# google-research/rigl

Hardware: AMD Instinct MI355X
Metric: images/sec/node, ResNet-50 80% ERK RigL step (higher is better)
Workload: dtype bf16

## Files before the change

rigl_amd/csrc/bn.hip:

```cpp
#include "common.hpp"

namespace rigl {
namespace kbn {

constexpr int THREADS = 256;
constexpr int MAX_PARTS = 512;

__device__ __forceinline__ float bf_lo(uint32_t w) { return __uint_as_float(w << 16); }
__device__ __forceinline__ float bf_hi(uint32_t w) { return __uint_as_float(w & 0xFFFF0000u); }
__device__ __forceinline__ uint32_t f2bf(float f) {
  uint32_t u = __float_as_uint(f);
  if ((u & 0x7FFFFFFFu) > 0x7F800000u) return (u >> 16) | 0x40u;
  u += 0x7FFFu + ((u >> 16) & 1u);
  return u >> 16;
}
typedef __attribute__((ext_vector_type(2))) __bf16 bf16x2_t;
typedef __attribute__((ext_vector_type(2))) float f32x2_t;
__device__ __forceinline__ uint32_t pack2(float a, float b) {
  const f32x2_t v = {a, b};
  return __builtin_bit_cast(uint32_t, __builtin_convertvector(v, bf16x2_t));
}
__device__ __forceinline__ void unpack8(const uint4& v, float f[8]) {
  f[0] = bf_lo(v.x); f[1] = bf_hi(v.x); f[2] = bf_lo(v.y); f[3] = bf_hi(v.y);
  f[4] = bf_lo(v.z); f[5] = bf_hi(v.z); f[6] = bf_lo(v.w); f[7] = bf_hi(v.w);
}

typedef unsigned int u32x4_t __attribute__((ext_vector_type(4)));
__device__ __forceinline__ void st16(uint16_t* p, const uint4& v, int nt) {
  if (nt) { const u32x4_t t = {v.x, v.y, v.z, v.w}; __builtin_nontemporal_store(t, reinterpret_cast<u32x4_t*>(p)); }
  else *reinterpret_cast<uint4*>(p) = v;
}
__device__ __forceinline__ uint4 ld16(const uint16_t* p, int nt) {
  if (nt > 1) { const u32x4_t t = __builtin_nontemporal_load(reinterpret_cast<const u32x4_t*>(p)); return make_uint4(t.x, t.y, t.z, t.w); }
  return *reinterpret_cast<const uint4*>(p);
}

struct Geom {
  int nt;
  int il;
  int64_t M;
  int C, cg;
  int tpr, rpb;
  int parts;
  int64_t rows_per_part;
  int fixed;
};

__device__ __forceinline__ void ld8f(const float* __restrict__ p, float (&o)[8]) {
  const float4 a = *reinterpret_cast<const float4*>(p), b = *reinterpret_cast<const float4*>(p + 4);
  o[0] = a.x; o[1] = a.y; o[2] = a.z; o[3] = a.w; o[4] = b.x; o[5] = b.y; o[6] = b.z; o[7] = b.w;
}

__device__ __forceinline__ float pivot3(float a, float b, float c) { return fmaxf(fminf(a, b), fminf(fmaxf(a, b), c)); }

template <int MODE, bool RELU, int MSK>
__global__ __launch_bounds__(THREADS) void k_reduce(Geom G, const uint16_t* __restrict__ x, const uint16_t* __restrict__ y,
                                                    const uint8_t* __restrict__ mbits,
                                                    const uint16_t* __restrict__ dy, const float* __restrict__ mean,
                                                    const float* __restrict__ invstd, const float* __restrict__ scale,
                                                    const float* __restrict__ shift, float* __restrict__ partial) {
  __shared__ float red[THREADS][17];
  const int tx = threadIdx.x % G.tpr, ty = threadIdx.x / G.tpr;
  const int cgi = blockIdx.y * G.tpr + tx;
  const bool c_ok = cgi < G.cg;
  const int64_t r0 = (int64_t)blockIdx.x * G.rows_per_part;
  int64_t r1 = r0 + G.rows_per_part;
  if (r1 > G.M) r1 = G.M;
  float q0[8], q1[8], mu[8], is[8], sc[8], sh[8];
#pragma unroll
  for (int j = 0; j < 8; ++j) { q0[j] = q1[j] = 0.f; mu[j] = is[j] = sc[j] = sh[j] = 0.f; }
  if (MODE == 1 && c_ok) {
#pragma unroll
    for (int j = 0; j < 8; ++j) {
      mu[j] = mean[cgi * 8 + j]; is[j] = invstd[cgi * 8 + j];
      if (RELU && MSK == 0) { sc[j] = scale[cgi * 8 + j]; sh[j] = shift[cgi * 8 + j]; }
    }
  }
  if (MODE == 0 && c_ok) {
    float pa[8], pb[8], pc[8];
    unpack8(*reinterpret_cast<const uint4*>(x + (int64_t)cgi * 8), pa);
    unpack8(*reinterpret_cast<const uint4*>(x + (G.M / 2) * G.C + (int64_t)cgi * 8), pb);
    unpack8(*reinterpret_cast<const uint4*>(x + (G.M - 1) * G.C + (int64_t)cgi * 8), pc);
#pragma unroll
    for (int j = 0; j < 8; ++j) mu[j] = pivot3(pa[j], pb[j], pc[j]);
  }
  if (c_ok) {
    const int64_t rb = G.il ? (int64_t)blockIdx.x * G.rpb + ty : r0 + ty, re = G.il ? G.M : r1;
    const int64_t rstep = G.il ? (int64_t)G.parts * G.rpb : (int64_t)G.rpb;
#pragma unroll 2
    for (int64_t r = rb; r < re; r += rstep) {
      const int64_t off = r * G.C + (int64_t)cgi * 8;
      float xv[8];
      unpack8(*reinterpret_cast<const uint4*>(x + off), xv);
      if (MODE == 0) {
#pragma unroll
        for (int j = 0; j < 8; ++j) { const float d = xv[j] - mu[j]; q0[j] += d; q1[j] = fmaf(d, d, q1[j]); }
      } else {
        float dv[8], yv[8];
        unpack8(*reinterpret_cast<const uint4*>(dy + off), dv);
        uint32_t mb = 0u;
        if (RELU && MSK == 1) unpack8(*reinterpret_cast<const uint4*>(y + off), yv);
        if (RELU && MSK == 2) mb = mbits[r * G.cg + cgi];
#pragma unroll
        for (int j = 0; j < 8; ++j) {
          bool on = true;
          if (RELU) on = MSK == 1 ? (yv[j] > 0.f) : (MSK == 2 ? ((mb >> j) & 1u) != 0u : (fmaf(xv[j], sc[j], sh[j]) > 0.f));
          const float dz = on ? dv[j] : 0.f;
          q0[j] += dz;
          q1[j] = fmaf(dz, (xv[j] - mu[j]) * is[j], q1[j]);
        }
      }
    }
  }
  float own[16];
#pragma unroll
  for (int j = 0; j < 8; ++j) { own[j] = q0[j]; own[8 + j] = q1[j]; red[threadIdx.x][j] = q0[j]; red[threadIdx.x][8 + j] = q1[j]; }
  __syncthreads();
  for (int s = G.rpb >> 1; s > 0; s >>= 1) {
    if (ty < s) {
      float oth[16];
#pragma unroll
      for (int j = 0; j < 16; ++j) oth[j] = red[threadIdx.x + s * G.tpr][j];
#pragma unroll
      for (int j = 0; j < 16; ++j) own[j] += oth[j];
      if (s > 1) {
#pragma unroll
        for (int j = 0; j < 16; ++j) red[threadIdx.x][j] = own[j];
      }
    }
    if (s > 1) __syncthreads();
  }
  if (ty == 0 && c_ok) {
    float* p = partial + ((int64_t)blockIdx.x * 2) * G.C + cgi * 8;
#pragma unroll
    for (int j = 0; j < 8; ++j) { p[j] = own[j]; p[G.C + j] = own[8 + j]; }
  }
}

template <int CL>
__device__ __forceinline__ void sum_partials(const Geom& G, const float* __restrict__ partial, double& s0, double& s1,
                                             int& c, bool& leader) {
  constexpr int PL = THREADS / CL;
  __shared__ double acc[2][PL][CL + 1];
  const int cl = threadIdx.x % CL, pl = threadIdx.x / CL;
  c = blockIdx.x * CL + cl;
  double a0 = 0.0, a1 = 0.0;
  if (c < G.C) {
#ifndef RIGL_BN_FIN_FLIGHT
#define RIGL_BN_FIN_FLIGHT 16
#endif
    constexpr int FLIGHT = RIGL_BN_FIN_FLIGHT;
    for (int p0 = pl; p0 < G.parts; p0 += PL * FLIGHT) {
      float v0[FLIGHT], v1[FLIGHT];
#pragma unroll
      for (int j = 0; j < FLIGHT; ++j) {
        const int p = p0 + j * PL;
        const int pc = p < G.parts ? p : G.parts - 1;
        const float l0 = partial[((int64_t)pc * 2) * G.C + c], l1 = partial[((int64_t)pc * 2 + 1) * G.C + c];
        v0[j] = p < G.parts ? l0 : 0.f;
        v1[j] = p < G.parts ? l1 : 0.f;
      }
#pragma unroll
      for (int j = 0; j < FLIGHT; ++j) { a0 += (double)v0[j]; a1 += (double)v1[j]; }
    }
  }
  acc[0][pl][cl] = a0; acc[1][pl][cl] = a1;
  __syncthreads();
  leader = pl == 0 && c < G.C;
  s0 = s1 = 0.0;
  if constexpr (CL == 1) {
    __shared__ double acc2[2][16];
    if (threadIdx.x < 16) {
      double t0 = 0.0, t1 = 0.0;
#pragma unroll
      for (int k = 0; k < 16; ++k) { t0 += acc[0][threadIdx.x * 16 + k][0]; t1 += acc[1][threadIdx.x * 16 + k][0]; }
      acc2[0][threadIdx.x] = t0; acc2[1][threadIdx.x] = t1;
    }
    __syncthreads();
    if (leader) {
#pragma unroll
      for (int k = 0; k < 16; ++k) { s0 += acc2[0][k]; s1 += acc2[1][k]; }
    }
  } else if (leader) {
#pragma unroll 8
    for (int k = 0; k < PL; ++k) { s0 += acc[0][k][cl]; s1 += acc[1][k][cl]; }
  }
}

template <int CL>
__global__ __launch_bounds__(THREADS) void k_fwd_finalize(Geom G, const float* __restrict__ partial,
                                                           const uint16_t* __restrict__ x ,
                                                           const float* __restrict__ gamma, const float* __restrict__ beta,
                                                           float* __restrict__ running_mean, float* __restrict__ running_var,
                                                           float momentum, float eps, float* __restrict__ save_mean,
                                                           float* __restrict__ save_invstd, float* __restrict__ scale,
                                                           float* __restrict__ shift) {
  double s0, s1; int c; bool leader;
  sum_partials<CL>(G, partial, s0, s1, c, leader);
  if (!leader) return;
  const double m = (double)G.M;
  double k = 0.0;
  if (x) {
    const float a = __uint_as_float((uint32_t)x[c] << 16), b = __uint_as_float((uint32_t)x[(G.M / 2) * G.C + c] << 16),
                e = __uint_as_float((uint32_t)x[(G.M - 1) * G.C + c] << 16);
    k = (double)pivot3(a, b, e);
  }
  const double dm = s0 / m;
  const double mean = k + dm;
  double var = s1 / m - dm * dm;
  if (var < 0.0) var = 0.0;
  const float invstd = (float)(1.0 / sqrt(var + (double)eps));
  save_mean[c] = (float)mean;
  save_invstd[c] = invstd;
  const float sc = gamma[c] * invstd;
  scale[c] = sc;
  shift[c] = beta[c] - (float)mean * sc;
  if (running_mean) {
    const double unbiased = G.M > 1 ? var * m / (m - 1.0) : var;
    running_mean[c] = (1.f - momentum) * running_mean[c] + momentum * (float)mean;
    running_var[c] = (1.f - momentum) * running_var[c] + momentum * (float)unbiased;
  }
}

template <bool RELU, bool HAS_RES>
__global__ __launch_bounds__(THREADS) void k_fwd_apply(Geom G, const uint16_t* __restrict__ x, const uint16_t* __restrict__ res,
                                                        const float* __restrict__ scale, const float* __restrict__ shift,
                                                        uint16_t* __restrict__ y, uint8_t* __restrict__ mbits) {
  extern __shared__ __attribute__((aligned(16))) float prm[];
  const bool fixed = G.fixed != 0;
  float psc[8], psh[8];
  if (fixed) {
    const int c0 = (int)(((int64_t)blockIdx.x * THREADS + threadIdx.x) % G.cg) * 8;
    ld8f(scale + c0, psc); ld8f(shift + c0, psh);
  } else {
    for (int i = threadIdx.x; i < G.C; i += THREADS) { prm[i] = scale[i]; prm[G.C + i] = shift[i]; }
    __syncthreads();
  }
  const int64_t total = G.M * G.cg;
  const int64_t stride = (int64_t)gridDim.x * THREADS;
  for (int64_t i = (int64_t)blockIdx.x * THREADS + threadIdx.x; i < total; i += stride) {
    if (!fixed) {
      const int cgi = (int)(i % G.cg);
#pragma unroll
      for (int j = 0; j < 8; ++j) { psc[j] = prm[cgi * 8 + j]; psh[j] = prm[G.C + cgi * 8 + j]; }
    }
    float xv[8], rv[8];
    unpack8(ld16(x + i * 8, G.nt), xv);
    if (HAS_RES) unpack8(ld16(res + i * 8, G.nt), rv);
    float o[8];
#pragma unroll
    for (int j = 0; j < 8; ++j) {
      float v = fmaf(xv[j], psc[j], psh[j]);
      if (HAS_RES) v += rv[j];
      o[j] = RELU ? fmaxf(v, 0.f) : v;
    }
    uint4 out;
    out.x = pack2(o[0], o[1]); out.y = pack2(o[2], o[3]); out.z = pack2(o[4], o[5]); out.w = pack2(o[6], o[7]);
    st16(y + i * 8, out, G.nt);
    if (RELU && mbits) {
      uint32_t mb = 0u;
#pragma unroll
      for (int j = 0; j < 8; ++j) mb |= (o[j] > 0.f ? 1u : 0u) << j;
      mbits[i] = (uint8_t)mb;
    }
  }
}

template <int CL>
__global__ __launch_bounds__(THREADS) void k_bwd_finalize(Geom G, const float* __restrict__ partial,
                                                           const float* __restrict__ gamma, const float* __restrict__ invstd,
                                                           float* __restrict__ dgamma, float* __restrict__ dbeta,
                                                           float* __restrict__ coef ) {
  double s0, s1; int c; bool leader;
  sum_partials<CL>(G, partial, s0, s1, c, leader);
  if (!leader) return;
  dbeta[c] = (float)s0;
  dgamma[c] = (float)s1;
  coef[c] = gamma[c] * invstd[c];
  coef[G.C + c] = (float)(s0 / (double)G.M);
  coef[2 * G.C + c] = (float)(s1 / (double)G.M);
}

template <bool RELU, int MSK, bool HAS_DRES>
__global__ __launch_bounds__(THREADS) void k_bwd_apply(Geom G, const uint16_t* __restrict__ x, const uint16_t* __restrict__ y,
                                                        const uint8_t* __restrict__ mbits,
                                                        const uint16_t* __restrict__ dy, const float* __restrict__ mean,
                                                        const float* __restrict__ invstd, const float* __restrict__ scale,
                                                        const float* __restrict__ shift, const float* __restrict__ coef,
                                                        uint16_t* __restrict__ dx, uint16_t* __restrict__ dres) {
  extern __shared__ __attribute__((aligned(16))) float prm[];
  const bool fixed = G.fixed != 0;
  float pm[8], pis[8], pa[8], pb[8], pc[8], psc[8], psh[8];
  if (fixed) {
    const int c0 = (int)(((int64_t)blockIdx.x * THREADS + threadIdx.x) % G.cg) * 8;
    ld8f(mean + c0, pm); ld8f(invstd + c0, pis);
    ld8f(coef + c0, pa); ld8f(coef + G.C + c0, pb); ld8f(coef + 2 * G.C + c0, pc);
    if (RELU && MSK == 0) { ld8f(scale + c0, psc); ld8f(shift + c0, psh); }
  } else {
    for (int i = threadIdx.x; i < G.C; i += THREADS) {
      prm[i] = mean[i]; prm[G.C + i] = invstd[i];
      prm[2 * G.C + i] = coef[i]; prm[3 * G.C + i] = coef[G.C + i]; prm[4 * G.C + i] = coef[2 * G.C + i];
      if (RELU && MSK == 0) { prm[5 * G.C + i] = scale[i]; prm[6 * G.C + i] = shift[i]; }
    }
    __syncthreads();
  }
  const int64_t total = G.M * G.cg;
  const int64_t stride = (int64_t)gridDim.x * THREADS;
  for (int64_t i = (int64_t)blockIdx.x * THREADS + threadIdx.x; i < total; i += stride) {
    if (!fixed) {
      const int c0 = (int)(i % G.cg) * 8;
#pragma unroll
      for (int j = 0; j < 8; ++j) {
        pm[j] = prm[c0 + j]; pis[j] = prm[G.C + c0 + j]; pa[j] = prm[2 * G.C + c0 + j]; pb[j] = prm[3 * G.C + c0 + j];
        pc[j] = prm[4 * G.C + c0 + j];
        if (RELU && MSK == 0) { psc[j] = prm[5 * G.C + c0 + j]; psh[j] = prm[6 * G.C + c0 + j]; }
      }
    }
    float xv[8], dv[8], yv[8];
    unpack8(ld16(x + i * 8, G.nt), xv);
    unpack8(ld16(dy + i * 8, G.nt), dv);
    uint32_t mb = 0u;
    if (RELU && MSK == 1) unpack8(*reinterpret_cast<const uint4*>(y + i * 8), yv);
    if (RELU && MSK == 2) mb = mbits[i];
    float o[8], z[8];
#pragma unroll
    for (int j = 0; j < 8; ++j) {
      bool on = true;
      if (RELU) on = MSK == 1 ? (yv[j] > 0.f) : (MSK == 2 ? ((mb >> j) & 1u) != 0u : (fmaf(xv[j], psc[j], psh[j]) > 0.f));
      const float dz = on ? dv[j] : 0.f;
      o[j] = bn_bwd_dx(dz, xv[j], pm[j], pis[j], pa[j], pb[j], pc[j]);
      z[j] = dz;
    }
    uint4 out;
    out.x = pack2(o[0], o[1]); out.y = pack2(o[2], o[3]); out.z = pack2(o[4], o[5]); out.w = pack2(o[6], o[7]);
    st16(dx + i * 8, out, G.nt);
    if (HAS_DRES) {
      out.x = pack2(z[0], z[1]); out.y = pack2(z[2], z[3]); out.z = pack2(z[4], z[5]); out.w = pack2(z[6], z[7]);
      st16(dres + i * 8, out, G.nt);
    }
  }
}

template <bool RELU>
__global__ __launch_bounds__(THREADS) void k_fwd_apply_pair(Geom G, const uint16_t* __restrict__ x, const uint16_t* __restrict__ x2,
                                                             const float* __restrict__ scale, const float* __restrict__ shift,
                                                             const float* __restrict__ scale2, const float* __restrict__ shift2,
                                                             uint16_t* __restrict__ y, uint8_t* __restrict__ mbits) {
  extern __shared__ __attribute__((aligned(16))) float prm[];
  const bool fixed = G.fixed != 0;
  float p0[8], p1[8], p2[8], p3[8];
  if (fixed) {
    const int c0 = (int)(((int64_t)blockIdx.x * THREADS + threadIdx.x) % G.cg) * 8;
    ld8f(scale + c0, p0); ld8f(shift + c0, p1); ld8f(scale2 + c0, p2); ld8f(shift2 + c0, p3);
  } else {
    for (int i = threadIdx.x; i < G.C; i += THREADS) {
      prm[i] = scale[i]; prm[G.C + i] = shift[i]; prm[2 * G.C + i] = scale2[i]; prm[3 * G.C + i] = shift2[i];
    }
    __syncthreads();
  }
  const int64_t total = G.M * G.cg;
  const int64_t stride = (int64_t)gridDim.x * THREADS;
  for (int64_t i = (int64_t)blockIdx.x * THREADS + threadIdx.x; i < total; i += stride) {
    if (!fixed) {
      const int c0 = (int)(i % G.cg) * 8;
#pragma unroll
      for (int j = 0; j < 8; ++j) { p0[j] = prm[c0 + j]; p1[j] = prm[G.C + c0 + j]; p2[j] = prm[2 * G.C + c0 + j]; p3[j] = prm[3 * G.C + c0 + j]; }
    }
    float xv[8], rv[8];
    unpack8(ld16(x + i * 8, G.nt), xv);
    unpack8(ld16(x2 + i * 8, G.nt), rv);
    float o[8];
#pragma unroll
    for (int j = 0; j < 8; j += 2) {
      const uint32_t pk = pack2(fmaf(rv[j], p2[j], p3[j]), fmaf(rv[j + 1], p2[j + 1], p3[j + 1]));
      float v0 = fmaf(xv[j], p0[j], p1[j]);
      float v1 = fmaf(xv[j + 1], p0[j + 1], p1[j + 1]);
      v0 += bf_lo(pk); v1 += bf_hi(pk);
      o[j] = RELU ? fmaxf(v0, 0.f) : v0;
      o[j + 1] = RELU ? fmaxf(v1, 0.f) : v1;
    }
    uint4 out;
    out.x = pack2(o[0], o[1]); out.y = pack2(o[2], o[3]); out.z = pack2(o[4], o[5]); out.w = pack2(o[6], o[7]);
    st16(y + i * 8, out, G.nt);
    if (RELU && mbits) {
      uint32_t mb = 0u;
#pragma unroll
      for (int j = 0; j < 8; ++j) mb |= (o[j] > 0.f ? 1u : 0u) << j;
      mbits[i] = (uint8_t)mb;
    }
  }
}

__global__ __launch_bounds__(THREADS) void k_reduce_pair(Geom G, const uint16_t* __restrict__ x, const uint16_t* __restrict__ x2,
                                                          const uint8_t* __restrict__ mbits, const uint16_t* __restrict__ dy,
                                                          const float* __restrict__ mean, const float* __restrict__ invstd,
                                                          const float* __restrict__ mean2, const float* __restrict__ invstd2,
                                                          float* __restrict__ partial, float* __restrict__ partial2) {
  __shared__ float red[THREADS][25];
  const int tx = threadIdx.x % G.tpr, ty = threadIdx.x / G.tpr;
  const int cgi = blockIdx.y * G.tpr + tx;
  const bool c_ok = cgi < G.cg;
  const int64_t r0 = (int64_t)blockIdx.x * G.rows_per_part;
  int64_t r1 = r0 + G.rows_per_part;
  if (r1 > G.M) r1 = G.M;
  float q0[8], q1[8], q2[8], mu[8], is[8], mu2[8], is2[8];
#pragma unroll
  for (int j = 0; j < 8; ++j) { q0[j] = q1[j] = q2[j] = 0.f; mu[j] = is[j] = mu2[j] = is2[j] = 0.f; }
  if (c_ok) {
#pragma unroll
    for (int j = 0; j < 8; ++j) {
      mu[j] = mean[cgi * 8 + j]; is[j] = invstd[cgi * 8 + j]; mu2[j] = mean2[cgi * 8 + j]; is2[j] = invstd2[cgi * 8 + j];
    }
    const int64_t rb = G.il ? (int64_t)blockIdx.x * G.rpb + ty : r0 + ty, re = G.il ? G.M : r1;
    const int64_t rstep = G.il ? (int64_t)G.parts * G.rpb : (int64_t)G.rpb;
#pragma unroll 2
    for (int64_t r = rb; r < re; r += rstep) {
      const int64_t off = r * G.C + (int64_t)cgi * 8;
      float xv[8], x2v[8], dv[8];
      unpack8(*reinterpret_cast<const uint4*>(x + off), xv);
      unpack8(*reinterpret_cast<const uint4*>(x2 + off), x2v);
      unpack8(*reinterpret_cast<const uint4*>(dy + off), dv);
      const uint32_t mb = mbits[r * G.cg + cgi];
#pragma unroll
      for (int j = 0; j < 8; ++j) {
        const float dz = ((mb >> j) & 1u) != 0u ? dv[j] : 0.f;
        q0[j] += dz;
        q1[j] = fmaf(dz, (xv[j] - mu[j]) * is[j], q1[j]);
        q2[j] = fmaf(dz, (x2v[j] - mu2[j]) * is2[j], q2[j]);
      }
    }
  }
  float own[24];
#pragma unroll
  for (int j = 0; j < 8; ++j) {
    own[j] = q0[j]; own[8 + j] = q1[j]; own[16 + j] = q2[j];
    red[threadIdx.x][j] = q0[j]; red[threadIdx.x][8 + j] = q1[j]; red[threadIdx.x][16 + j] = q2[j];
  }
  __syncthreads();
  for (int s = G.rpb >> 1; s > 0; s >>= 1) {
    if (ty < s) {
      float oth[24];
#pragma unroll
      for (int j = 0; j < 24; ++j) oth[j] = red[threadIdx.x + s * G.tpr][j];
#pragma unroll
      for (int j = 0; j < 24; ++j) own[j] += oth[j];
      if (s > 1) {
#pragma unroll
        for (int j = 0; j < 24; ++j) red[threadIdx.x][j] = own[j];
      }
    }
    if (s > 1) __syncthreads();
  }
  if (ty == 0 && c_ok) {
    float* p = partial + ((int64_t)blockIdx.x * 2) * G.C + cgi * 8;
    float* p2 = partial2 + ((int64_t)blockIdx.x * 2) * G.C + cgi * 8;
#pragma unroll
    for (int j = 0; j < 8; ++j) {
      p[j] = own[j]; p[G.C + j] = own[8 + j];
      p2[j] = own[j]; p2[G.C + j] = own[16 + j];
    }
  }
}

struct FinSet { const float* partial; const float* gamma; const float* invstd; float* dgamma; float* dbeta; float* coef; };

template <int CL>
__global__ __launch_bounds__(THREADS) void k_bwd_finalize_pair(Geom G, FinSet s0, FinSet s1) {
  const FinSet& f = blockIdx.y == 0 ? s0 : s1;
  double a0, a1; int c; bool leader;
  sum_partials<CL>(G, f.partial, a0, a1, c, leader);
  if (!leader) return;
  f.dbeta[c] = (float)a0;
  f.dgamma[c] = (float)a1;
  f.coef[c] = f.gamma[c] * f.invstd[c];
  f.coef[G.C + c] = (float)(a0 / (double)G.M);
  f.coef[2 * G.C + c] = (float)(a1 / (double)G.M);
}

__global__ __launch_bounds__(THREADS) void k_bwd_apply_pair(Geom G, const uint16_t* __restrict__ x, const uint16_t* __restrict__ x2,
                                                             const uint8_t* __restrict__ mbits, const uint16_t* __restrict__ dy,
                                                             const float* __restrict__ mean, const float* __restrict__ invstd,
                                                             const float* __restrict__ mean2, const float* __restrict__ invstd2,
                                                             const float* __restrict__ coef, const float* __restrict__ coef2,
                                                             uint16_t* __restrict__ dx, uint16_t* __restrict__ dx2) {
  extern __shared__ __attribute__((aligned(16))) float prm[];
  const bool fixed = G.fixed != 0;
  float q[10][8];
  if (fixed) {
    const int c0 = (int)(((int64_t)blockIdx.x * THREADS + threadIdx.x) % G.cg) * 8;
    ld8f(mean + c0, q[0]); ld8f(invstd + c0, q[1]); ld8f(coef + c0, q[2]); ld8f(coef + G.C + c0, q[3]); ld8f(coef + 2 * G.C + c0, q[4]);
    ld8f(mean2 + c0, q[5]); ld8f(invstd2 + c0, q[6]); ld8f(coef2 + c0, q[7]); ld8f(coef2 + G.C + c0, q[8]); ld8f(coef2 + 2 * G.C + c0, q[9]);
  } else {
    for (int i = threadIdx.x; i < G.C; i += THREADS) {
      prm[i] = mean[i]; prm[G.C + i] = invstd[i];
      prm[2 * G.C + i] = coef[i]; prm[3 * G.C + i] = coef[G.C + i]; prm[4 * G.C + i] = coef[2 * G.C + i];
      prm[5 * G.C + i] = mean2[i]; prm[6 * G.C + i] = invstd2[i];
      prm[7 * G.C + i] = coef2[i]; prm[8 * G.C + i] = coef2[G.C + i]; prm[9 * G.C + i] = coef2[2 * G.C + i];
    }
    __syncthreads();
  }
  const int64_t total = G.M * G.cg;
  const int64_t stride = (int64_t)gridDim.x * THREADS;
  for (int64_t i = (int64_t)blockIdx.x * THREADS + threadIdx.x; i < total; i += stride) {
    if (!fixed) {
      const int c0 = (int)(i % G.cg) * 8;
#pragma unroll
      for (int k = 0; k < 10; ++k)
#pragma unroll
        for (int j = 0; j < 8; ++j) q[k][j] = prm[k * G.C + c0 + j];
    }
    float xv[8], x2v[8], dv[8];
    unpack8(ld16(x + i * 8, G.nt), xv);
    unpack8(ld16(x2 + i * 8, G.nt), x2v);
    unpack8(ld16(dy + i * 8, G.nt), dv);
    const uint32_t mb = mbits[i];
    float o[8], o2[8];
#pragma unroll
    for (int j = 0; j < 8; ++j) {
      const float dz = ((mb >> j) & 1u) != 0u ? dv[j] : 0.f;
      const float xh = (xv[j] - q[0][j]) * q[1][j];
      o[j] = q[2][j] * (dz - q[3][j] - xh * q[4][j]);
      const float xh2 = (x2v[j] - q[5][j]) * q[6][j];
      o2[j] = q[7][j] * (dz - q[8][j] - xh2 * q[9][j]);
    }
    uint4 out;
    out.x = pack2(o[0], o[1]); out.y = pack2(o[2], o[3]); out.z = pack2(o[4], o[5]); out.w = pack2(o[6], o[7]);
    st16(dx + i * 8, out, G.nt);
    out.x = pack2(o2[0], o2[1]); out.y = pack2(o2[2], o2[3]); out.z = pack2(o2[4], o2[5]); out.w = pack2(o2[6], o2[7]);
    st16(dx2 + i * 8, out, G.nt);
  }
}

constexpr int INFER_BATCH = 64;
struct InferBatch {
  RiglBnInferItem it[INFER_BATCH];
  int32_t blk_begin[INFER_BATCH + 1];
  int32_t count;
};
__global__ __launch_bounds__(THREADS) void k_infer_params(InferBatch B) {
  int i = 0;
  while (i + 1 < B.count && (int)blockIdx.x >= B.blk_begin[i + 1]) ++i;
  const RiglBnInferItem& t = B.it[i];
  const int c = ((int)blockIdx.x - B.blk_begin[i]) * THREADS + (int)threadIdx.x;
  if (c >= t.c) return;
  const float invstd = (float)(1.0 / sqrt((double)t.moving_variance[c] + (double)t.eps));
  const float sc = t.gamma[c] * invstd;
  t.scale_shift[c] = sc;
  t.scale_shift[t.c + c] = t.beta[c] - t.moving_mean[c] * sc;
}

static Geom make_geom(int64_t m, int c) {
  Geom g;
  g.nt = (int64_t)m * c * 2 >= (int64_t)RIGL_TUNE("bn_nt_mb", 0) * (1 << 20) ? RIGL_TUNE("bn_nt", 2) : 0;
  g.il = RIGL_TUNE("bn_il", 1);
  g.fixed = 0;
  g.M = m; g.C = c; g.cg = c / 8;
  int tpr = 1;
  while (tpr < g.cg && tpr < THREADS) tpr <<= 1;
  g.tpr = tpr; g.rpb = THREADS / tpr;
#ifndef RIGL_BN_ROWS_PER_LANE
#define RIGL_BN_ROWS_PER_LANE 8
#endif
  int64_t parts = (m + (int64_t)g.rpb * RIGL_BN_ROWS_PER_LANE - 1) / ((int64_t)g.rpb * RIGL_BN_ROWS_PER_LANE);
  const int64_t cap = RIGL_TUNE("bn_max_parts", MAX_PARTS);
  if (parts > cap) parts = cap;
  if (parts < 1) parts = 1;
  int64_t rpp = (m + parts - 1) / parts;
  rpp = (rpp + g.rpb - 1) / g.rpb * g.rpb;
  g.rows_per_part = rpp;
  g.parts = (int)((m + rpp - 1) / rpp);
  return g;
}

static unsigned apply_grid(Geom& g) {
#ifndef RIGL_BN_APPLY_PER_THREAD
#define RIGL_BN_APPLY_PER_THREAD 2
#endif
#ifndef RIGL_BN_APPLY_CAP
#define RIGL_BN_APPLY_CAP 16384
#endif
  int64_t b = (g.M * g.cg + THREADS * RIGL_BN_APPLY_PER_THREAD - 1) / (THREADS * RIGL_BN_APPLY_PER_THREAD);
  if (b > RIGL_BN_APPLY_CAP) b = RIGL_BN_APPLY_CAP;
  if (b < 1) b = 1;
  g.fixed = (RIGL_TUNE("bn_regs", 1) != 0 && (b * THREADS) % g.cg == 0) ? 1 : 0;
  return (unsigned)b;
}

void launch_bwd_finalize(int64_t m, int c, const float* partial, int parts, const float* gamma, const float* invstd,
                         float* dgamma, float* dbeta, float* coef, hipStream_t st) {
  Geom g = make_geom(m, c);
  g.parts = parts;
  if (parts > MAX_PARTS)
    hipLaunchKernelGGL(k_bwd_finalize<4>, dim3((unsigned)((c + 3) / 4)), dim3(THREADS), 0, st, g, partial, gamma, invstd,
                       dgamma, dbeta, coef);
  else
    hipLaunchKernelGGL(k_bwd_finalize<16>, dim3((unsigned)((c + 15) / 16)), dim3(THREADS), 0, st, g, partial, gamma, invstd,
                       dgamma, dbeta, coef);
}

static int fwd_statistics(Geom& g, int32_t c, const rigl_bf16* x, const float* gamma, const float* beta,
                          float* running_mean, float* running_var, float momentum, float eps, float* save_mean,
                          float* save_invstd, float* save_scale, float* save_shift, const float* stats,
                          int32_t stats_parts, void* workspace, size_t workspace_bytes, hipStream_t st) {
  const float* partial = stats;
  if (!stats) {
    const size_t need = rigl_bn_workspace_bytes(g.M, c);
    if (!workspace || workspace_bytes < need) return fail(RIGL_EWORKSPACE, "rigl_bn_fwd: workspace %zu < %zu", workspace_bytes, need);
    float* ws_partial = static_cast<float*>(workspace);
    dim3 rgrid((unsigned)g.parts, (unsigned)((g.cg + g.tpr - 1) / g.tpr));
    hipLaunchKernelGGL((k_reduce<0, false, 0>), rgrid, dim3(THREADS), 0, st, g, x, nullptr, nullptr, nullptr, nullptr, nullptr,
                       nullptr, nullptr, ws_partial);
    partial = ws_partial;
  } else {
    g.parts = stats_parts;
  }
  if (g.parts > 1024 && RIGL_TUNE("bn_fin1", 1) != 0)
    hipLaunchKernelGGL(k_fwd_finalize<1>, dim3((unsigned)c), dim3(THREADS), 0, st, g, partial, stats ? nullptr : reinterpret_cast<const uint16_t*>(x), gamma,
                       beta, running_mean, running_var, momentum, eps, save_mean, save_invstd, save_scale, save_shift);
  else if (g.parts > 256)
    hipLaunchKernelGGL(k_fwd_finalize<4>, dim3((unsigned)((c + 3) / 4)), dim3(THREADS), 0, st, g, partial, stats ? nullptr : reinterpret_cast<const uint16_t*>(x), gamma,
                       beta, running_mean, running_var, momentum, eps, save_mean, save_invstd, save_scale, save_shift);
  else
    hipLaunchKernelGGL(k_fwd_finalize<16>, dim3((unsigned)((c + 15) / 16)), dim3(THREADS), 0, st, g, partial, stats ? nullptr : reinterpret_cast<const uint16_t*>(x), gamma,
                       beta, running_mean, running_var, momentum, eps, save_mean, save_invstd, save_scale, save_shift);
  return RIGL_OK;
}

}
}

extern "C" {

size_t rigl_bn_workspace_bytes(int64_t m, int32_t c) {
  if (m <= 0 || c <= 0) return 0;
  rigl::kbn::Geom g = rigl::kbn::make_geom(m, c);
  return rigl::align_up((size_t)g.parts * 2 * c * 4, 256) + rigl::align_up((size_t)3 * c * 4, 256);
}

int rigl_bn_fwd_stats(int64_t m, int32_t c, const rigl_bf16* x, const rigl_bf16* residual, const float* gamma,
                      const float* beta, float* running_mean, float* running_var, float momentum, float eps,
                      int32_t relu, rigl_bf16* y, float* save_mean, float* save_invstd, float* save_scale,
                      float* save_shift, const float* stats, int32_t stats_parts, uint8_t* relu_bits,
                      void* workspace, size_t workspace_bytes, rigl_stream_t stream) {
  using namespace rigl;
  using namespace rigl::kbn;
  if (m <= 0 || c <= 0 || !x || !gamma || !beta || !y || !save_mean || !save_invstd || !save_scale || !save_shift)
    return fail(RIGL_EINVAL, "rigl_bn_fwd: bad arguments");
  if (c % 8) return fail(RIGL_EUNSUPPORTED, "rigl_bn_fwd: channels %% 8 != 0");
  if (2 * (size_t)c * 4 > 65536) return fail(RIGL_EUNSUPPORTED, "rigl_bn_fwd: too many channels for the LDS parameter cache");
  if (stats && stats_parts <= 0) return fail(RIGL_EINVAL, "rigl_bn_fwd_stats: stats_parts must be positive");
  hipStream_t st = as_stream(stream);
  Geom g = make_geom(m, c);
  int rc = fwd_statistics(g, c, x, gamma, beta, running_mean, running_var, momentum, eps, save_mean, save_invstd,
                          save_scale, save_shift, stats, stats_parts, workspace, workspace_bytes, st);
  if (rc) return rc;
  dim3 agrid(apply_grid(g));
  const size_t lds = g.fixed ? 0 : (size_t)2 * c * 4;
  if (relu && residual) hipLaunchKernelGGL((k_fwd_apply<true, true>), agrid, dim3(THREADS), lds, st, g, x, residual, save_scale, save_shift, y, relu_bits);
  else if (relu) hipLaunchKernelGGL((k_fwd_apply<true, false>), agrid, dim3(THREADS), lds, st, g, x, residual, save_scale, save_shift, y, relu_bits);
  else if (residual) hipLaunchKernelGGL((k_fwd_apply<false, true>), agrid, dim3(THREADS), lds, st, g, x, residual, save_scale, save_shift, y, nullptr);
  else hipLaunchKernelGGL((k_fwd_apply<false, false>), agrid, dim3(THREADS), lds, st, g, x, residual, save_scale, save_shift, y, nullptr);
  RIGL_CHECK_LAUNCH("rigl_bn_fwd");
  return RIGL_OK;
}

int rigl_bn_fwd(int64_t m, int32_t c, const rigl_bf16* x, const rigl_bf16* residual, const float* gamma,
                const float* beta, float* running_mean, float* running_var, float momentum, float eps, int32_t relu,
                rigl_bf16* y, float* save_mean, float* save_invstd, float* save_scale, float* save_shift,
                void* workspace, size_t workspace_bytes, rigl_stream_t stream) {
  return rigl_bn_fwd_stats(m, c, x, residual, gamma, beta, running_mean, running_var, momentum, eps, relu, y, save_mean,
                           save_invstd, save_scale, save_shift, nullptr, 0, nullptr, workspace, workspace_bytes, stream);
}

int rigl_bn_fwd_statistics(int64_t m, int32_t c, const rigl_bf16* x, const float* gamma, const float* beta,
                           float* running_mean, float* running_var, float momentum, float eps, float* save_mean,
                           float* save_invstd, float* save_scale, float* save_shift, const float* stats,
                           int32_t stats_parts, void* workspace, size_t workspace_bytes, rigl_stream_t stream) {
  using namespace rigl;
  using namespace rigl::kbn;
  if (m <= 0 || c <= 0 || (!x && !stats) || !gamma || !beta || !save_mean || !save_invstd || !save_scale || !save_shift)
    return fail(RIGL_EINVAL, "rigl_bn_fwd_statistics: bad arguments");
  if (c % 8) return fail(RIGL_EUNSUPPORTED, "rigl_bn_fwd_statistics: channels %% 8 != 0");
  if (stats && stats_parts <= 0) return fail(RIGL_EINVAL, "rigl_bn_fwd_statistics: stats_parts must be positive");
  Geom g = make_geom(m, c);
  int rc = fwd_statistics(g, c, x, gamma, beta, running_mean, running_var, momentum, eps, save_mean, save_invstd,
                          save_scale, save_shift, stats, stats_parts, workspace, workspace_bytes, as_stream(stream));
  if (rc) return rc;
  RIGL_CHECK_LAUNCH("rigl_bn_fwd_statistics");
  return RIGL_OK;
}

int rigl_bn_add_bn_fwd(int64_t m, int32_t c, const rigl_bf16* x, const rigl_bf16* x2, const float* scale2,
                       const float* shift2, const float* gamma, const float* beta, float* running_mean,
                       float* running_var, float momentum, float eps, int32_t relu, rigl_bf16* y, float* save_mean,
                       float* save_invstd, float* save_scale, float* save_shift, const float* stats,
                       int32_t stats_parts, uint8_t* relu_bits, void* workspace, size_t workspace_bytes,
                       rigl_stream_t stream) {
  using namespace rigl;
  using namespace rigl::kbn;
  if (m <= 0 || c <= 0 || !x || !x2 || !scale2 || !shift2 || !gamma || !beta || !y || !save_mean || !save_invstd ||
      !save_scale || !save_shift)
    return fail(RIGL_EINVAL, "rigl_bn_add_bn_fwd: bad arguments");
  if (c % 8) return fail(RIGL_EUNSUPPORTED, "rigl_bn_add_bn_fwd: channels %% 8 != 0");
  if (4 * (size_t)c * 4 > 65536) return fail(RIGL_EUNSUPPORTED, "rigl_bn_add_bn_fwd: too many channels for the LDS parameter cache");
  if (stats && stats_parts <= 0) return fail(RIGL_EINVAL, "rigl_bn_add_bn_fwd: stats_parts must be positive");
  hipStream_t st = as_stream(stream);
  Geom g = make_geom(m, c);
  int rc = fwd_statistics(g, c, x, gamma, beta, running_mean, running_var, momentum, eps, save_mean, save_invstd,
                          save_scale, save_shift, stats, stats_parts, workspace, workspace_bytes, st);
  if (rc) return rc;
  dim3 agrid(apply_grid(g));
  const size_t lds = g.fixed ? 0 : (size_t)4 * c * 4;
  if (relu) hipLaunchKernelGGL(k_fwd_apply_pair<true>, agrid, dim3(THREADS), lds, st, g, x, x2, save_scale, save_shift, scale2, shift2, y, relu_bits);
  else hipLaunchKernelGGL(k_fwd_apply_pair<false>, agrid, dim3(THREADS), lds, st, g, x, x2, save_scale, save_shift, scale2, shift2, y, nullptr);
  RIGL_CHECK_LAUNCH("rigl_bn_add_bn_fwd");
  return RIGL_OK;
}

size_t rigl_bn_add_bn_bwd_workspace_bytes(int64_t m, int32_t c) { return 2 * rigl_bn_workspace_bytes(m, c); }

int rigl_bn_add_bn_bwd(int64_t m, int32_t c, const rigl_bf16* x, const rigl_bf16* x2, const uint8_t* relu_bits,
                       const rigl_bf16* dy, const float* gamma, const float* save_mean, const float* save_invstd,
                       const float* gamma2, const float* save_mean2, const float* save_invstd2, rigl_bf16* dx,
                       rigl_bf16* dx2, float* dgamma, float* dbeta, float* dgamma2, float* dbeta2, void* workspace,
                       size_t workspace_bytes, rigl_stream_t stream) {
  using namespace rigl;
  using namespace rigl::kbn;
  if (m <= 0 || c <= 0 || !x || !x2 || !relu_bits || !dy || !gamma || !save_mean || !save_invstd || !gamma2 || !save_mean2 ||
      !save_invstd2 || !dx || !dx2 || !dgamma || !dbeta || !dgamma2 || !dbeta2)
    return fail(RIGL_EINVAL, "rigl_bn_add_bn_bwd: bad arguments");
  if (c % 8) return fail(RIGL_EUNSUPPORTED, "rigl_bn_add_bn_bwd: channels %% 8 != 0");
  const size_t lds = (size_t)10 * c * 4;
  if (lds > 160 * 1024 - 1024) return fail(RIGL_EUNSUPPORTED, "rigl_bn_add_bn_bwd: too many channels for the LDS parameter cache");
  const size_t need = rigl_bn_add_bn_bwd_workspace_bytes(m, c);
  if (!workspace || workspace_bytes < need) return fail(RIGL_EWORKSPACE, "rigl_bn_add_bn_bwd: workspace %zu < %zu", workspace_bytes, need);
  static const bool big_lds = hipFuncSetAttribute(reinterpret_cast<const void*>(&k_bwd_apply_pair),
                                                  hipFuncAttributeMaxDynamicSharedMemorySize, 159 * 1024) == hipSuccess;
  if (lds > 65536 && !big_lds) return fail(RIGL_ELAUNCH, "rigl_bn_add_bn_bwd: cannot raise the dynamic LDS limit");
  hipStream_t st = as_stream(stream);
  Geom g = make_geom(m, c);
  const size_t half = rigl_bn_workspace_bytes(m, c);
  const size_t part_bytes = align_up((size_t)g.parts * 2 * c * 4, 256);
  char* w0 = static_cast<char*>(workspace);
  float* partial = reinterpret_cast<float*>(w0);
  float* coef = reinterpret_cast<float*>(w0 + part_bytes);
  float* partial2 = reinterpret_cast<float*>(w0 + half);
  float* coef2 = reinterpret_cast<float*>(w0 + half + part_bytes);
  dim3 rgrid((unsigned)g.parts, (unsigned)((g.cg + g.tpr - 1) / g.tpr));
  hipLaunchKernelGGL(k_reduce_pair, rgrid, dim3(THREADS), 0, st, g, x, x2, relu_bits, dy, save_mean, save_invstd, save_mean2,
                     save_invstd2, partial, partial2);
  const FinSet f0 = {partial, gamma, save_invstd, dgamma, dbeta, coef};
  const FinSet f1 = {partial2, gamma2, save_invstd2, dgamma2, dbeta2, coef2};
  hipLaunchKernelGGL(k_bwd_finalize_pair<16>, dim3((unsigned)((c + 15) / 16), 2), dim3(THREADS), 0, st, g, f0, f1);
  const dim3 pgrid(apply_grid(g));
  hipLaunchKernelGGL(k_bwd_apply_pair, pgrid, dim3(THREADS), g.fixed ? 0 : lds, st, g, x, x2, relu_bits, dy, save_mean, save_invstd,
                     save_mean2, save_invstd2, coef, coef2, dx, dx2);
  RIGL_CHECK_LAUNCH("rigl_bn_add_bn_bwd");
  return RIGL_OK;
}

static int bn_bwd_impl(int64_t m, int32_t c, const rigl_bf16* x, const rigl_bf16* y, const uint8_t* relu_bits,
                       const rigl_bf16* dy, const float* gamma,
                       const float* save_mean, const float* save_invstd, const float* save_scale, const float* save_shift,
                       int32_t relu, rigl_bf16* dx, rigl_bf16* dresidual, float* dgamma, float* dbeta,
                       const float* stats, int32_t stats_parts, float* coef_out, void* workspace,
                       size_t workspace_bytes, rigl_stream_t stream) {
  using namespace rigl;
  using namespace rigl::kbn;
  if (m <= 0 || c <= 0 || !x || !dy || !gamma || !save_mean || !save_invstd || (!dx && !coef_out) || !dgamma || !dbeta)
    return fail(RIGL_EINVAL, "rigl_bn_bwd: bad arguments");
  if (c % 8) return fail(RIGL_EUNSUPPORTED, "rigl_bn_bwd: channels %% 8 != 0");
  if (relu && !y && !relu_bits && (!save_scale || !save_shift))
    return fail(RIGL_EINVAL, "rigl_bn_bwd: relu needs y, relu_bits or scale/shift");
  if (7 * (size_t)c * 4 > 65536) return fail(RIGL_EUNSUPPORTED, "rigl_bn_bwd: too many channels for the LDS parameter cache");
  if (stats && stats_parts <= 0) return fail(RIGL_EINVAL, "rigl_bn_bwd_stats: stats_parts must be positive");
  const size_t need = rigl_bn_workspace_bytes(m, c);
  if (!workspace || workspace_bytes < need) return fail(RIGL_EWORKSPACE, "rigl_bn_bwd: workspace %zu < %zu", workspace_bytes, need);
  hipStream_t st = as_stream(stream);
  Geom g = make_geom(m, c);
  float* partial = static_cast<float*>(workspace);
  float* coef = coef_out ? coef_out : reinterpret_cast<float*>(static_cast<char*>(workspace) + align_up((size_t)g.parts * 2 * c * 4, 256));
  dim3 rgrid((unsigned)g.parts, (unsigned)((g.cg + g.tpr - 1) / g.tpr));
  const int msk = relu_bits ? 2 : (y ? 1 : 0);
  const float* red = partial;
  if (stats) {
    red = stats;
    g.parts = stats_parts;
  } else {
#define RIGL_BWD_REDUCE(R, K) hipLaunchKernelGGL((k_reduce<1, R, K>), rgrid, dim3(THREADS), 0, st, g, x, y, relu_bits, dy, save_mean, save_invstd, save_scale, save_shift, partial)
    if (!relu) RIGL_BWD_REDUCE(false, 0);
    else if (msk == 2) RIGL_BWD_REDUCE(true, 2);
    else if (msk == 1) RIGL_BWD_REDUCE(true, 1);
    else RIGL_BWD_REDUCE(true, 0);
#undef RIGL_BWD_REDUCE
  }
  if (g.parts > MAX_PARTS)
    hipLaunchKernelGGL(k_bwd_finalize<4>, dim3((unsigned)((c + 3) / 4)), dim3(THREADS), 0, st, g, red, gamma,
                       save_invstd, dgamma, dbeta, coef);
  else
    hipLaunchKernelGGL(k_bwd_finalize<16>, dim3((unsigned)((c + 15) / 16)), dim3(THREADS), 0, st, g, red, gamma,
                       save_invstd, dgamma, dbeta, coef);
  if (coef_out) {
    RIGL_CHECK_LAUNCH("rigl_bn_bwd_reduce");
    return RIGL_OK;
  }
  dim3 agrid(apply_grid(g));
  const size_t lds = g.fixed ? 0 : (size_t)7 * c * 4;
#define RIGL_BWD_APPLY(R, K, D) hipLaunchKernelGGL((k_bwd_apply<R, K, D>), agrid, dim3(THREADS), lds, st, g, x, y, relu_bits, dy, save_mean, save_invstd, save_scale, save_shift, coef, dx, dresidual)
  const bool dres = dresidual != nullptr;
  if (!relu) { if (dres) RIGL_BWD_APPLY(false, 0, true); else RIGL_BWD_APPLY(false, 0, false); }
  else if (msk == 2) { if (dres) RIGL_BWD_APPLY(true, 2, true); else RIGL_BWD_APPLY(true, 2, false); }
  else if (msk == 1) { if (dres) RIGL_BWD_APPLY(true, 1, true); else RIGL_BWD_APPLY(true, 1, false); }
  else { if (dres) RIGL_BWD_APPLY(true, 0, true); else RIGL_BWD_APPLY(true, 0, false); }
#undef RIGL_BWD_APPLY
  RIGL_CHECK_LAUNCH("rigl_bn_bwd");
  return RIGL_OK;
}

int rigl_bn_bwd_stats(int64_t m, int32_t c, const rigl_bf16* x, const rigl_bf16* y, const uint8_t* relu_bits,
                      const rigl_bf16* dy, const float* gamma,
                      const float* save_mean, const float* save_invstd, const float* save_scale, const float* save_shift,
                      int32_t relu, rigl_bf16* dx, rigl_bf16* dresidual, float* dgamma, float* dbeta,
                      const float* stats, int32_t stats_parts, void* workspace,
                      size_t workspace_bytes, rigl_stream_t stream) {
  return bn_bwd_impl(m, c, x, y, relu_bits, dy, gamma, save_mean, save_invstd, save_scale, save_shift, relu, dx, dresidual, dgamma,
                     dbeta, stats, stats_parts, nullptr, workspace, workspace_bytes, stream);
}

int rigl_bn_bwd_reduce(int64_t m, int32_t c, const rigl_bf16* x, const uint8_t* relu_bits, const rigl_bf16* dy, const float* gamma,
                       const float* save_mean, const float* save_invstd, int32_t relu, float* dgamma, float* dbeta, float* coef,
                       void* workspace, size_t workspace_bytes, rigl_stream_t stream) {
  if (!coef) return rigl::fail(RIGL_EINVAL, "rigl_bn_bwd_reduce: coef is required");
  if (relu && !relu_bits) return rigl::fail(RIGL_EINVAL, "rigl_bn_bwd_reduce: relu needs relu_bits");
  return bn_bwd_impl(m, c, x, nullptr, relu ? relu_bits : nullptr, dy, gamma, save_mean, save_invstd, nullptr, nullptr, relu, nullptr,
                     nullptr, dgamma, dbeta, nullptr, 0, coef, workspace, workspace_bytes, stream);
}

int rigl_bn_bwd(int64_t m, int32_t c, const rigl_bf16* x, const rigl_bf16* y, const uint8_t* relu_bits,
                const rigl_bf16* dy, const float* gamma,
                const float* save_mean, const float* save_invstd, const float* save_scale, const float* save_shift,
                int32_t relu, rigl_bf16* dx, rigl_bf16* dresidual, float* dgamma, float* dbeta, void* workspace,
                size_t workspace_bytes, rigl_stream_t stream) {
  return rigl_bn_bwd_stats(m, c, x, y, relu_bits, dy, gamma, save_mean, save_invstd, save_scale, save_shift, relu, dx,
                           dresidual, dgamma, dbeta, nullptr, 0, workspace, workspace_bytes, stream);
}

int rigl_bn_infer_params_batched(const RiglBnInferItem* items, int32_t n_items, rigl_stream_t stream) {
  using namespace rigl;
  using namespace rigl::kbn;
  if (n_items < 0 || (n_items > 0 && !items)) return fail(RIGL_EINVAL, "rigl_bn_infer_params_batched: bad arguments");
  for (int i = 0; i < n_items; ++i) {
    const RiglBnInferItem& t = items[i];
    if (t.c < 0 || (t.c > 0 && (!t.gamma || !t.beta || !t.moving_mean || !t.moving_variance || !t.scale_shift)))
      return fail(RIGL_EINVAL, "rigl_bn_infer_params_batched: item %d: bad channels / NULL tensor", i);
  }
  hipStream_t st = as_stream(stream);
  for (int b = 0; b < n_items; b += INFER_BATCH) {
    InferBatch B;
    B.count = 0;
    int32_t blk = 0;
    for (int i = b; i < n_items && i < b + INFER_BATCH; ++i) {
      if (items[i].c == 0) continue;
      B.it[B.count] = items[i];
      B.blk_begin[B.count] = blk;
      blk += (items[i].c + THREADS - 1) / THREADS;
      ++B.count;
    }
    B.blk_begin[B.count] = blk;
    if (B.count) hipLaunchKernelGGL(k_infer_params, dim3((unsigned)blk), dim3(THREADS), 0, st, B);
  }
  RIGL_CHECK_LAUNCH("rigl_bn_infer_params_batched");
  return RIGL_OK;
}

int rigl_bn_apply(int64_t m, int32_t c, const rigl_bf16* x, const rigl_bf16* residual, const float* scale_shift, int32_t relu,
                  rigl_bf16* y, rigl_stream_t stream) {
  using namespace rigl;
  using namespace rigl::kbn;
  if (m <= 0 || c <= 0 || !x || !scale_shift || !y) return fail(RIGL_EINVAL, "rigl_bn_apply: bad arguments");
  if (c % 8) return fail(RIGL_EUNSUPPORTED, "rigl_bn_apply: channels %% 8 != 0");
  if (2 * (size_t)c * 4 > 65536) return fail(RIGL_EUNSUPPORTED, "rigl_bn_apply: too many channels for the LDS parameter cache");
  hipStream_t st = as_stream(stream);
  Geom g = make_geom(m, c);
  dim3 agrid(apply_grid(g));
  const size_t lds = g.fixed ? 0 : (size_t)2 * c * 4;
  const float* sc = scale_shift;
  const float* sh = scale_shift + c;
  if (relu && residual) hipLaunchKernelGGL((k_fwd_apply<true, true>), agrid, dim3(THREADS), lds, st, g, x, residual, sc, sh, y, nullptr);
  else if (relu) hipLaunchKernelGGL((k_fwd_apply<true, false>), agrid, dim3(THREADS), lds, st, g, x, residual, sc, sh, y, nullptr);
  else if (residual) hipLaunchKernelGGL((k_fwd_apply<false, true>), agrid, dim3(THREADS), lds, st, g, x, residual, sc, sh, y, nullptr);
  else hipLaunchKernelGGL((k_fwd_apply<false, false>), agrid, dim3(THREADS), lds, st, g, x, residual, sc, sh, y, nullptr);
  RIGL_CHECK_LAUNCH("rigl_bn_apply");
  return RIGL_OK;
}

int rigl_bn_apply_pair(int64_t m, int32_t c, const rigl_bf16* x, const rigl_bf16* x2, const float* scale_shift,
                       const float* scale_shift2, int32_t relu, rigl_bf16* y, rigl_stream_t stream) {
  using namespace rigl;
  using namespace rigl::kbn;
  if (m <= 0 || c <= 0 || !x || !x2 || !scale_shift || !scale_shift2 || !y) return fail(RIGL_EINVAL, "rigl_bn_apply_pair: bad arguments");
  if (c % 8) return fail(RIGL_EUNSUPPORTED, "rigl_bn_apply_pair: channels %% 8 != 0");
  if (4 * (size_t)c * 4 > 65536) return fail(RIGL_EUNSUPPORTED, "rigl_bn_apply_pair: too many channels for the LDS parameter cache");
  hipStream_t st = as_stream(stream);
  Geom g = make_geom(m, c);
  dim3 agrid(apply_grid(g));
  const size_t lds = g.fixed ? 0 : (size_t)4 * c * 4;
  if (relu) hipLaunchKernelGGL(k_fwd_apply_pair<true>, agrid, dim3(THREADS), lds, st, g, x, x2, scale_shift, scale_shift + c, scale_shift2, scale_shift2 + c, y, nullptr);
  else hipLaunchKernelGGL(k_fwd_apply_pair<false>, agrid, dim3(THREADS), lds, st, g, x, x2, scale_shift, scale_shift + c, scale_shift2, scale_shift2 + c, y, nullptr);
  RIGL_CHECK_LAUNCH("rigl_bn_apply_pair");
  return RIGL_OK;
}

}
```

Measured before the change: 12630.

## Add software-pipelined BN reduce kernel with optional 4-channel-per-thread variant

Adds a new templated BN statistics and backward-reduction kernel that double-buffers row loads in registers, issuing the next row's loads before accumulating the current one, with scheduling barriers to hold that order. The default arm uses 4 channels per thread with doubled block size for more memory-level parallelism. It replaces the forward stats reduce, the single BN backward reduce and the paired add+BN backward reduce. This is meant to hide global load latency in these memory-bound reductions, at the cost of more registers and a clamped tail row being loaded redundantly.

```diff
diff --git a/rigl_amd/csrc/bn.hip b/rigl_amd/csrc/bn.hip
--- a/rigl_amd/csrc/bn.hip
+++ b/rigl_amd/csrc/bn.hip
@@ -5,6 +5,9 @@
 
 constexpr int THREADS = 256;
 constexpr int MAX_PARTS = 512;
+#ifndef RIGL_BN_REDUCE_DEFAULT
+#define RIGL_BN_REDUCE_DEFAULT 2
+#endif
 
 __device__ __forceinline__ float bf_lo(uint32_t w) { return __uint_as_float(w << 16); }
 __device__ __forceinline__ float bf_hi(uint32_t w) { return __uint_as_float(w & 0xFFFF0000u); }
@@ -458,6 +461,173 @@
     for (int j = 0; j < 8; ++j) {
       p[j] = own[j]; p[G.C + j] = own[8 + j];
       p2[j] = own[j]; p2[G.C + j] = own[16 + j];
+    }
+  }
+}
+
+typedef unsigned int u32x2_t __attribute__((ext_vector_type(2)));
+template <int NCH> struct ChVec;
+template <> struct ChVec<8> { typedef u32x4_t type; };
+template <> struct ChVec<4> { typedef u32x2_t type; };
+__device__ __forceinline__ void unpack_ch(const u32x4_t& v, float (&f)[8]) {
+  f[0] = bf_lo(v.x); f[1] = bf_hi(v.x); f[2] = bf_lo(v.y); f[3] = bf_hi(v.y);
+  f[4] = bf_lo(v.z); f[5] = bf_hi(v.z); f[6] = bf_lo(v.w); f[7] = bf_hi(v.w);
+}
+__device__ __forceinline__ void unpack_ch(const u32x2_t& v, float (&f)[4]) {
+  f[0] = bf_lo(v.x); f[1] = bf_hi(v.x); f[2] = bf_lo(v.y); f[3] = bf_hi(v.y);
+}
+
+struct ReduceArgs {
+  const uint16_t *x, *x2, *y, *dy;
+  const uint8_t* mbits;
+};
+
+template <int MODE, bool RELU, int MSK, int NCH>
+struct RowRegs {
+  static constexpr bool HAS_Y = MODE == 1 && RELU && MSK == 1;
+  static constexpr bool HAS_BITS = MODE == 2 || (MODE == 1 && RELU && MSK == 2);
+  typedef typename ChVec<NCH>::type V;
+  V x, x2, y, dy;
+  uint8_t mb;
+
+  __device__ __forceinline__ void load(const Geom& G, const ReduceArgs& a, int64_t r, int ci) {
+    const int64_t off = r * G.C + (int64_t)ci * NCH;
+    x = *reinterpret_cast<const V*>(a.x + off);
+    if (MODE == 2) x2 = *reinterpret_cast<const V*>(a.x2 + off);
+    if (MODE >= 1) dy = *reinterpret_cast<const V*>(a.dy + off);
+    if (HAS_Y) y = *reinterpret_cast<const V*>(a.y + off);
+    if (HAS_BITS) mb = a.mbits[r * G.cg + (NCH == 8 ? ci : ci >> 1)];
+  }
+
+  __device__ __forceinline__ void add(int bit0, float (&q0)[NCH], float (&q1)[NCH], float (&q2)[NCH], const float (&mu)[NCH],
+                                      const float (&is)[NCH], const float (&pa)[NCH], const float (&pb)[NCH]) const {
+    float xv[NCH];
+    unpack_ch(x, xv);
+    if (MODE == 0) {
+#pragma unroll
+      for (int j = 0; j < NCH; ++j) { const float d = xv[j] - mu[j]; q0[j] += d; q1[j] = fmaf(d, d, q1[j]); }
+    } else {
+      float dv[NCH], yv[NCH], x2v[NCH];
+      unpack_ch(dy, dv);
+      if (HAS_Y) unpack_ch(y, yv);
+      if (MODE == 2) unpack_ch(x2, x2v);
+      const uint32_t bits = HAS_BITS ? (uint32_t)mb >> bit0 : 0u;
+#pragma unroll
+      for (int j = 0; j < NCH; ++j) {
+        bool on = true;
+        if (HAS_BITS) on = ((bits >> j) & 1u) != 0u;
+        else if (HAS_Y) on = yv[j] > 0.f;
+        else if (RELU) on = fmaf(xv[j], pa[j], pb[j]) > 0.f;
+        const float dz = on ? dv[j] : 0.f;
+        q0[j] += dz;
+        q1[j] = fmaf(dz, (xv[j] - mu[j]) * is[j], q1[j]);
+        if (MODE == 2) q2[j] = fmaf(dz, (x2v[j] - pa[j]) * pb[j], q2[j]);
+      }
+    }
+  }
+};
+
+__device__ __forceinline__ void pin_sums(float (&q)[8]) {
+  asm volatile("" : "+v"(q[0]), "+v"(q[1]), "+v"(q[2]), "+v"(q[3]), "+v"(q[4]), "+v"(q[5]), "+v"(q[6]), "+v"(q[7]));
+}
+__device__ __forceinline__ void pin_sums(float (&q)[4]) { asm volatile("" : "+v"(q[0]), "+v"(q[1]), "+v"(q[2]), "+v"(q[3])); }
+
+template <int MODE, bool RELU, int MSK, int NCH>
+__device__ __forceinline__ void reduce_rows(const Geom& G, const ReduceArgs& a, int ci, int64_t rb, int64_t re, int64_t rstep,
+                                            float (&q0)[NCH], float (&q1)[NCH], float (&q2)[NCH], const float (&mu)[NCH],
+                                            const float (&is)[NCH], const float (&pa)[NCH], const float (&pb)[NCH]) {
+  const int bit0 = NCH == 8 ? 0 : (ci & 1) * 4;
+  const int64_t last = G.M - 1;
+  RowRegs<MODE, RELU, MSK, NCH> A, B;
+  const int64_t n = rb < re ? (re - rb + rstep - 1) / rstep : 0;
+  int64_t r = rb;
+  A.load(G, a, r < last ? r : last, ci);
+  for (int64_t t = 2; t <= n; t += 2) {
+    r += rstep;
+    B.load(G, a, r < last ? r : last, ci);
+    __builtin_amdgcn_sched_barrier(0);
+    A.add(bit0, q0, q1, q2, mu, is, pa, pb);
+    pin_sums(q0); pin_sums(q1); if (MODE == 2) pin_sums(q2);
+    r += rstep;
+    A.load(G, a, r < last ? r : last, ci);
+    __builtin_amdgcn_sched_barrier(0);
+    B.add(bit0, q0, q1, q2, mu, is, pa, pb);
+    pin_sums(q0); pin_sums(q1); if (MODE == 2) pin_sums(q2);
+  }
+  if (n & 1) A.add(bit0, q0, q1, q2, mu, is, pa, pb);
+}
+
+template <int NQ, int NT>
+__device__ __forceinline__ void combine_row_lanes(const Geom& G, int ty, float (&own)[NQ]) {
+  __shared__ float red[NT][NQ + 1];
+#pragma unroll
+  for (int j = 0; j < NQ; ++j) red[threadIdx.x][j] = own[j];
+  __syncthreads();
+  for (int s = G.rpb >> 1; s > 0; s >>= 1) {
+    if (ty < s) {
+      float oth[NQ];
+#pragma unroll
+      for (int j = 0; j < NQ; ++j) oth[j] = red[threadIdx.x + s * G.tpr][j];
+#pragma unroll
+      for (int j = 0; j < NQ; ++j) own[j] += oth[j];
+      if (s > 1) {
+#pragma unroll
+        for (int j = 0; j < NQ; ++j) red[threadIdx.x][j] = own[j];
+      }
+    }
+    if (s > 1) __syncthreads();
+  }
+}
+
+template <int MODE, bool RELU, int MSK, int NCH>
+__global__ __launch_bounds__(THREADS * 8 / NCH) void k_reduce_pl(Geom G, ReduceArgs a, const float* __restrict__ mean,
+                                                                 const float* __restrict__ invstd, const float* __restrict__ pa_,
+                                                                 const float* __restrict__ pb_, float* __restrict__ partial,
+                                                                 float* __restrict__ partial2) {
+  constexpr int NT = THREADS * 8 / NCH, NQ = (MODE == 2 ? 3 : 2) * NCH;
+  const int tx = threadIdx.x % G.tpr, ty = threadIdx.x / G.tpr;
+  const int ci = blockIdx.y * G.tpr + tx;
+  const bool c_ok = ci < G.C / NCH;
+  float q0[NCH], q1[NCH], q2[NCH], mu[NCH], is[NCH], pa[NCH], pb[NCH];
+#pragma unroll
+  for (int j = 0; j < NCH; ++j) { q0[j] = q1[j] = q2[j] = 0.f; mu[j] = is[j] = pa[j] = pb[j] = 0.f; }
+  if (c_ok) {
+    if (MODE >= 1) {
+#pragma unroll
+      for (int j = 0; j < NCH; ++j) {
+        mu[j] = mean[ci * NCH + j]; is[j] = invstd[ci * NCH + j];
+        if (MODE == 2 || (RELU && MSK == 0)) { pa[j] = pa_[ci * NCH + j]; pb[j] = pb_[ci * NCH + j]; }
+      }
+    } else {
+      typedef typename ChVec<NCH>::type V;
+      float p0[NCH], p1[NCH], p2[NCH];
+      unpack_ch(*reinterpret_cast<const V*>(a.x + (int64_t)ci * NCH), p0);
+      unpack_ch(*reinterpret_cast<const V*>(a.x + (G.M / 2) * G.C + (int64_t)ci * NCH), p1);
+      unpack_ch(*reinterpret_cast<const V*>(a.x + (G.M - 1) * G.C + (int64_t)ci * NCH), p2);
+#pragma unroll
+      for (int j = 0; j < NCH; ++j) mu[j] = pivot3(p0[j], p1[j], p2[j]);
+    }
+    const int64_t r0 = (int64_t)blockIdx.x * G.rows_per_part;
+    const int64_t r1 = r0 + G.rows_per_part < G.M ? r0 + G.rows_per_part : G.M;
+    const int64_t rb = G.il ? (int64_t)blockIdx.x * G.rpb + ty : r0 + ty, re = G.il ? G.M : r1;
+    const int64_t rstep = G.il ? (int64_t)G.parts * G.rpb : (int64_t)G.rpb;
+    reduce_rows<MODE, RELU, MSK, NCH>(G, a, ci, rb, re, rstep, q0, q1, q2, mu, is, pa, pb);
+  }
+  float own[NQ];
+#pragma unroll
+  for (int j = 0; j < NCH; ++j) {
+    own[j] = q0[j]; own[NCH + j] = q1[j];
+    if constexpr (MODE == 2) own[2 * NCH + j] = q2[j];
+  }
+  combine_row_lanes<NQ, NT>(G, ty, own);
+  if (ty == 0 && c_ok) {
+    float* p = partial + ((int64_t)blockIdx.x * 2) * G.C + ci * NCH;
+#pragma unroll
+    for (int j = 0; j < NCH; ++j) { p[j] = own[j]; p[G.C + j] = own[NCH + j]; }
+    if constexpr (MODE == 2) {
+      float* p2 = partial2 + ((int64_t)blockIdx.x * 2) * G.C + ci * NCH;
+#pragma unroll
+      for (int j = 0; j < NCH; ++j) { p2[j] = own[j]; p2[G.C + j] = own[2 * NCH + j]; }
     }
   }
 }
@@ -586,6 +756,24 @@
   return (unsigned)b;
 }
 
+static int reduce_arm() {
+  const int k = RIGL_TUNE("bn_reduce", RIGL_BN_REDUCE_DEFAULT);
+  return k < 0 ? 0 : (k > 2 ? 2 : k);
+}
+
+template <int MODE, bool RELU, int MSK>
+static void launch_reduce_pl(int arm, const Geom& g, hipStream_t st, const ReduceArgs& a, const float* mean, const float* invstd,
+                             const float* pa, const float* pb, float* partial, float* partial2) {
+  const dim3 rgrid((unsigned)g.parts, (unsigned)((g.cg + g.tpr - 1) / g.tpr));
+  if (arm == 2) {
+    Geom h = g;
+    h.tpr = 2 * g.tpr;
+    hipLaunchKernelGGL((k_reduce_pl<MODE, RELU, MSK, 4>), rgrid, dim3(2 * THREADS), 0, st, h, a, mean, invstd, pa, pb, partial, partial2);
+  } else {
+    hipLaunchKernelGGL((k_reduce_pl<MODE, RELU, MSK, 8>), rgrid, dim3(THREADS), 0, st, g, a, mean, invstd, pa, pb, partial, partial2);
+  }
+}
+
 void launch_bwd_finalize(int64_t m, int c, const float* partial, int parts, const float* gamma, const float* invstd,
                          float* dgamma, float* dbeta, float* coef, hipStream_t st) {
   Geom g = make_geom(m, c);
@@ -608,8 +796,13 @@
     if (!workspace || workspace_bytes < need) return fail(RIGL_EWORKSPACE, "rigl_bn_fwd: workspace %zu < %zu", workspace_bytes, need);
     float* ws_partial = static_cast<float*>(workspace);
     dim3 rgrid((unsigned)g.parts, (unsigned)((g.cg + g.tpr - 1) / g.tpr));
-    hipLaunchKernelGGL((k_reduce<0, false, 0>), rgrid, dim3(THREADS), 0, st, g, x, nullptr, nullptr, nullptr, nullptr, nullptr,
-                       nullptr, nullptr, ws_partial);
+    if (const int arm = reduce_arm()) {
+      const ReduceArgs ra = {reinterpret_cast<const uint16_t*>(x), nullptr, nullptr, nullptr, nullptr};
+      launch_reduce_pl<0, false, 0>(arm, g, st, ra, nullptr, nullptr, nullptr, nullptr, ws_partial, nullptr);
+    } else {
+      hipLaunchKernelGGL((k_reduce<0, false, 0>), rgrid, dim3(THREADS), 0, st, g, x, nullptr, nullptr, nullptr, nullptr, nullptr,
+                         nullptr, nullptr, ws_partial);
+    }
     partial = ws_partial;
   } else {
     g.parts = stats_parts;
@@ -747,8 +940,14 @@
   float* partial2 = reinterpret_cast<float*>(w0 + half);
   float* coef2 = reinterpret_cast<float*>(w0 + half + part_bytes);
   dim3 rgrid((unsigned)g.parts, (unsigned)((g.cg + g.tpr - 1) / g.tpr));
-  hipLaunchKernelGGL(k_reduce_pair, rgrid, dim3(THREADS), 0, st, g, x, x2, relu_bits, dy, save_mean, save_invstd, save_mean2,
-                     save_invstd2, partial, partial2);
+  if (const int arm = reduce_arm()) {
+    const ReduceArgs ra = {reinterpret_cast<const uint16_t*>(x), reinterpret_cast<const uint16_t*>(x2), nullptr,
+                           reinterpret_cast<const uint16_t*>(dy), relu_bits};
+    launch_reduce_pl<2, true, 2>(arm, g, st, ra, save_mean, save_invstd, save_mean2, save_invstd2, partial, partial2);
+  } else {
+    hipLaunchKernelGGL(k_reduce_pair, rgrid, dim3(THREADS), 0, st, g, x, x2, relu_bits, dy, save_mean, save_invstd, save_mean2,
+                       save_invstd2, partial, partial2);
+  }
   const FinSet f0 = {partial, gamma, save_invstd, dgamma, dbeta, coef};
   const FinSet f1 = {partial2, gamma2, save_invstd2, dgamma2, dbeta2, coef2};
   hipLaunchKernelGGL(k_bwd_finalize_pair<16>, dim3((unsigned)((c + 15) / 16), 2), dim3(THREADS), 0, st, g, f0, f1);
@@ -787,7 +986,14 @@
     red = stats;
     g.parts = stats_parts;
   } else {
-#define RIGL_BWD_REDUCE(R, K) hipLaunchKernelGGL((k_reduce<1, R, K>), rgrid, dim3(THREADS), 0, st, g, x, y, relu_bits, dy, save_mean, save_invstd, save_scale, save_shift, partial)
+    const int arm = reduce_arm();
+    const ReduceArgs ra = {reinterpret_cast<const uint16_t*>(x), nullptr, reinterpret_cast<const uint16_t*>(y),
+                           reinterpret_cast<const uint16_t*>(dy), relu_bits};
+#define RIGL_BWD_REDUCE(R, K)                                                                                                  \
+  do {                                                                                                                         \
+    if (arm) launch_reduce_pl<1, R, K>(arm, g, st, ra, save_mean, save_invstd, save_scale, save_shift, partial, nullptr);       \
+    else hipLaunchKernelGGL((k_reduce<1, R, K>), rgrid, dim3(THREADS), 0, st, g, x, y, relu_bits, dy, save_mean, save_invstd, save_scale, save_shift, partial); \
+  } while (0)
     if (!relu) RIGL_BWD_REDUCE(false, 0);
     else if (msk == 2) RIGL_BWD_REDUCE(true, 2);
     else if (msk == 1) RIGL_BWD_REDUCE(true, 1);
```

New measurement: 12740 (median of 6 runs). No clear change (+0.9%).
